# sthagen/kubernetes-kubernetes

Hardware: AMD Instinct MI355X
Metric: pods scheduled/sec + node-evals/sec at 5k/100k nodes, 1/2/4/8 MI355X (higher is better)
Workload: dtype int64; 1 GPU; SchedulingBasic 5000 nodes / 1000 init pods / 491000 measured pods (BASELINE configs[1]); nodes=5000, percentageOfNodesToScore=100, plugins=default, parallelism=single

## Files before the change

### __graft_entry__.py

```python
import os
import subprocess
import sys

ROOT = os.path.dirname(os.path.abspath(__file__))
PKG = os.path.join(ROOT, "kubernetes-kubernetes_amd")
for p in (PKG, os.path.join(ROOT, "tests")):
    if p not in sys.path:
        sys.path.insert(0, p)


def _jobs():
    return str(min(16, os.cpu_count() or 4))


def build() -> None:
    env = dict(os.environ, PYTORCH_ROCM_ARCH="gfx950")
    subprocess.check_call(["make", "-j" + _jobs(), "-C", PKG, "ARCH=gfx950"], env=env)
    subprocess.check_call(["make", "-j" + _jobs(), "-C", os.path.join(ROOT, "oracle")], env=env)
    subprocess.check_call(["make", "-j" + _jobs(), "-C", os.path.join(ROOT, "tests", "asan")], env=env)
    import ksg
    from ksg import native
    native.load()


def smoke() -> None:
    from ksg.native import Scheduler
    from fuzz_gen import rand_cluster, rand_pod
    from oracle_binding import oracle

    rng, cfg, nodes, existing, names = rand_cluster(7, n_nodes=300, n_existing=60, cfg_index=0)
    g = Scheduler(dict(cfg, device=0))
    o = oracle(cfg)
    for b in (g, o):
        for n in nodes:
# ... 20 lines not shown
```

### include/ksg.h

```cpp
#ifndef KSG_H_
#define KSG_H_

#include <stddef.h>
#include <stdint.h>

#ifdef __cplusplus
extern "C" {
#endif

#define KSG_ABI_VERSION 3

#define KSG_OK 0
#define KSG_EINVAL (-1)
#define KSG_ENOTFOUND (-2)
#define KSG_EEXIST (-3)
#define KSG_EDEVICE (-4)
#define KSG_ENOTSUP (-5)
#define KSG_ENOMEM (-6)

#define KSG_CODE_SUCCESS 0
#define KSG_CODE_ERROR 1
#define KSG_CODE_UNSCHEDULABLE 2
#define KSG_CODE_UNSCHEDULABLE_AND_UNRESOLVABLE 3
#define KSG_CODE_WAIT 4
// ... 132 lines not shown

int ksg_debug_relayouts(const ksg_ctx *ctx, uint64_t *full, uint64_t *gather);

int ksg_debug_loop_stats(const ksg_ctx *ctx, uint64_t *give_ups, uint64_t *retries);

int ksg_debug_group_loop_kernel(char *buf, size_t cap);

int ksg_debug_lean_pods(const ksg_ctx *ctx, uint64_t *lean, uint64_t *general);

int ksg_debug_same_pods(const ksg_ctx *ctx, uint64_t *taken, uint64_t *not_taken);

int ksg_debug_compile_memo(const ksg_ctx *ctx, uint64_t *hits, uint64_t *misses);

int ksg_debug_same_carry(const ksg_ctx *ctx, uint64_t *loaded, uint64_t *filled);

int ksg_debug_sched_same(ksg_ctx *ctx, int32_t handle_a, int32_t handle_b);


int ksg_debug_resident_calls(const ksg_ctx *ctx, uint64_t *sched, uint64_t *agg, uint64_t *launch);

int ksg_debug_log_table(double *out, int32_t n);

int ksg_generation(const ksg_ctx *ctx, uint64_t *list_gen, uint64_t *events);

int ksg_debug_schedule_calls(ksg_ctx *ctx, const int32_t *handles, int32_t n, uint32_t flags, ksg_result *results,
                             double *us_per_call);

int ksg_debug_pod_resources(const char *pod_json, size_t len, int64_t *out, int32_t cap);

int ksg_debug_pod_signature(const char *config_json, size_t config_len, const char *pod_json, size_t pod_len, char *out,
// ... 14 lines not shown
```

### kubernetes-kubernetes_amd/csrc/common/desc.h

```cpp
#pragma once
#include <stddef.h>
#include <stdint.h>

#if defined(__HIP__) || defined(__HIPCC__)
#define KSG_HD __host__ __device__
#else
#define KSG_HD
#endif

namespace ksg {

constexpr int kNumPlugins = 10;
constexpr int kBlock = 256;
constexpr int kMaxScalar = 16;
constexpr int kPortSlots = 8;
constexpr int kMaxCons = 32;
constexpr int kMaxPodTerms = 64;
constexpr int kAggMaxCons = 8;
constexpr int kAggMaxTerms = 8;
constexpr int kMaxShards = 8;
constexpr int kBlobLds = 16384;
constexpr int kLoopMaxPods = 1024;
constexpr int kLoopMaxBlk = 2;

// ... 505 lines not shown
  uint32_t* fail;
  unsigned long long* stamps;
  const uint32_t* desc_bytes;
  unsigned long long* wstamps;
  int32_t give_up_at;
  int32_t wave_map;
  PodRing* ring;
  unsigned long long ring_idle;
  int32_t ring_ahead;
  int32_t split_eval;
  int32_t lean_select;
  unsigned long long* relay;
  int32_t* diag;
  unsigned long long* carry;
  uint32_t carry_tag, carry_expect;
};
constexpr int kGran = 16;
constexpr int kFailWords = 16;
constexpr int kFailBytes = kFailWords * 4;

constexpr int kSameScanWaves = 8, kSameCommitWaves = 8;
constexpr int kSameThreads = (kSameScanWaves + kSameCommitWaves) * 64;
constexpr int kSameSlots = 16;
constexpr int kSameMaxNodes = kSameSlots * kSameScanWaves * 64;
constexpr int kSameGroups = kSameMaxNodes / 64;
constexpr int kSameLdsBytes = kBlobLds + kSameMaxNodes * (8 + 1) + kSameGroups * 16 + kLoopMaxPods * (4 + 4 + 16) + 256;
constexpr int kSameSampledLdsBytes = kSameLdsBytes + kLoopMaxPods * (4 + 4) + 64;
static_assert(kSameLdsBytes <= 160 * 1024 && kSameSampledLdsBytes <= 160 * 1024,
              "k_sched_same: one workgroup's LDS (160 KiB per CU on gfx950)");
static_assert(kSameGroups <= 128, "k_sched_same: the group prefix scan holds two groups per lane");
constexpr int kSameCarryTot = 0, kSameCarryFx1 = kSameMaxNodes, kSameCarryBall0 = 2 * kSameMaxNodes,
              kSameCarryBall1 = kSameCarryBall0 + kSameGroups, kSameCarryTagWord = kSameCarryBall1 + kSameGroups;
constexpr int kSameCarryWords = kSameCarryTagWord + 1;
static_assert(kSameMaxNodes >= 5000, "k_sched_same: the flagship workload's nodes fit");

constexpr int kAggThreads = 512;
constexpr int kAggLocal = 4;
constexpr int kAggGWords = 1024;
constexpr int kAggLocalCons = 2;
constexpr int kAggPods = 5120;
constexpr int kAggTerms = 5120;
constexpr int kAggBlobLds = 8192;
// ... 160 lines not shown
```

### kubernetes-kubernetes_amd/csrc/hip/kernels.hip

```cpp
#include <hip/hip_ext.h>
#include <hip/hip_runtime.h>

#include <atomic>
#include <type_traits>

#include "device.hpp"

namespace ksg {

struct NodeCore {
  int64_t acpu, amem, aeph, rcpu, rmem, reph, nzcpu, nzmem;
  int32_t apods, npods;
  uint32_t flags, tlo, thi, ilo, ihi;
};
__device__ __forceinline__ const int32_t* nom_head(const uint8_t* tab) {
  return reinterpret_cast<const int32_t*>(tab + sizeof(NomHdr));
}
template <bool NOM = true>
__device__ __forceinline__ NodeCore load_core(const MirrorView& m, int i) {
  NodeCore c;
  c.acpu = m.alloc_cpu[i];
  c.amem = m.alloc_mem[i];
  c.aeph = m.alloc_eph[i];
  c.rcpu = m.req_cpu[i];
// ... 6525 lines not shown
  int32_t res_node[kLoopMaxPods];
  uint32_t res_F[kLoopMaxPods];
  int32_t slot[kLoopMaxPods], rot[kLoopMaxPods];
  unsigned long long wkey[2][kSameScanWaves];
  uint32_t wnode[2][kSameScanWaves];
  uint32_t arrive, arrive2, done, abort;
  uint8_t pend[kSameMaxNodes];
};
static_assert(sizeof(SameLds) <= (size_t)kSameLdsBytes, "k_sched_same: LDS layout (desc.h kSameLdsBytes)");
struct SameLdsSampled : SameLds {
  uint32_t res_rot[kLoopMaxPods];
  uint32_t res_proc[kLoopMaxPods];
  uint32_t wend[2][kSameScanWaves];
};
static_assert(sizeof(SameLdsSampled) <= (size_t)kSameSampledLdsBytes, "k_sched_same<1>: LDS layout (desc.h kSameSampledLdsBytes)");

__device__ __forceinline__ bool same_wait(SameLds& L, const uint32_t* word, uint32_t want, uint32_t* fail, int q, int what) {
  if ((int32_t)(__hip_atomic_load(word, __ATOMIC_ACQUIRE, __HIP_MEMORY_SCOPE_WORKGROUP) - want) >= 0) return true;
  const unsigned long long t_start = __builtin_amdgcn_s_memrealtime();
  for (uint32_t spins = 1;; ++spins) {
    if ((int32_t)(__hip_atomic_load(word, __ATOMIC_ACQUIRE, __HIP_MEMORY_SCOPE_WORKGROUP) - want) >= 0) return true;
    if ((spins & 63u) == 0u) {
      if (__hip_atomic_load(&L.abort, __ATOMIC_RELAXED, __HIP_MEMORY_SCOPE_WORKGROUP)) return false;
      if (__builtin_amdgcn_s_memrealtime() - t_start > 200000000ull) {
        if ((threadIdx.x & 63) == 0) {
          __hip_atomic_store(&L.abort, 1u, __ATOMIC_RELAXED, __HIP_MEMORY_SCOPE_WORKGROUP);
          __hip_atomic_store(fail + 1, (uint32_t)q, __ATOMIC_RELAXED, __HIP_MEMORY_SCOPE_AGENT);
          __hip_atomic_store(fail + 2, (uint32_t)what, __ATOMIC_RELAXED, __HIP_MEMORY_SCOPE_AGENT);
          __hip_atomic_store(fail + 3, (uint32_t)(threadIdx.x >> 6), __ATOMIC_RELAXED, __HIP_MEMORY_SCOPE_AGENT);
          __hip_atomic_store(fail + 4, 1u, __ATOMIC_RELAXED, __HIP_MEMORY_SCOPE_AGENT);
// ... 49 lines not shown
    for (int g = ct; g < kSameGroups; g += kSameThreads - kScanThreads) {
      cy[kSameCarryBall0 + g] = L.ball0[g];
      cy[kSameCarryBall1 + g] = L.ball1[g];
    }
  }
  __syncthreads();
  if (tid == 0) cy[kSameCarryTagWord] = (unsigned long long)lv.carry_tag;
}

__device__ __forceinline__ NodeEval same_eval(const MirrorView& m, NodeCore c, int k, const PodFast& pf, const uint8_t* base,
                                              const PodDesc& d, int i) {
  for (int a = 0; a < k; ++a) assume_core(c, d);
  return eval_core_fast<false>(m, c, bal2(c.rcpu, c.acpu, c.rmem, c.amem), pf, base, d, i);
}

template <int kSampled>
__global__ __launch_bounds__(kSameThreads) void k_sched_same(MirrorView m_, BatchView b_, LoopView lv_) {
  const LoopGroupArg& ka = *(const LoopGroupArg*)__builtin_amdgcn_kernarg_segment_ptr();
  const MirrorView& m = ka.m;
  const BatchView& b = ka.b;
  const LoopView& lv = ka.lv;
  __shared__ std::conditional_t<kSampled != 0, SameLdsSampled, SameLds> L;
  constexpr int kScanThreads = kSameScanWaves * 64;
  const int tid = (int)threadIdx.x, lane = tid & 63;
  const int wv = __builtin_amdgcn_readfirstlane(tid >> 6);
  const bool scan = wv < kSameScanWaves;
  const int npods = lv.npods;
  loop_entry_record(lv.fail, 0);
  const unsigned long long* cy = lv.carry;
  const bool carried = cy != nullptr && lv.carry_expect != 0u &&
                       (uint32_t)__builtin_amdgcn_readfirstlane((int)(uint32_t)cy[kSameCarryTagWord]) == lv.carry_expect;
  {
    const uint32_t off0 = b.desc_off[lv.first_pod];
    const uint4* src = reinterpret_cast<const uint4*>(b.descs + off0);
    uint4* dst = reinterpret_cast<uint4*>(L.blob);
    const uint32_t n16 = lv.desc_bytes[lv.first_pod] / 16u;
    for (uint32_t o = (uint32_t)tid; o < n16; o += (uint32_t)kSameThreads) dst[o] = src[o];
    for (int k = tid; k < npods; k += kSameThreads) {
      const PodDesc* pd = reinterpret_cast<const PodDesc*>(b.descs + b.desc_off[lv.first_pod + k]);
      L.slot[k] = pd->slot;
      L.rot[k] = pd->rot_start;
    }
    for (int k = tid; k < kSameGroups; k += kSameThreads) {
      L.ball0[k] = carried ? cy[kSameCarryBall0 + k] : 0ull;
      L.ball1[k] = carried ? cy[kSameCarryBall1 + k] : 0ull;
    }
    if (carried)
      for (int k = tid; k < m.n; k += kSameThreads) L.fx1[k] = (int64_t)cy[kSameCarryFx1 + k];
    for (int k = tid; k < kSameMaxNodes; k += kSameThreads) L.pend[k] = 0;
    if (tid == 0) L.arrive = L.arrive2 = L.done = L.abort = 0u;
  }
  __syncthreads();
  if (tid == 0) reinterpret_cast<PodDesc*>(L.blob)->slot = -1;
  __syncthreads();
  const uint8_t* base = L.blob;
  const PodDesc& d = *reinterpret_cast<const PodDesc*>(base);
// ... 25 lines not shown
      if (scan) {
        if constexpr (kSampled) tot[j] = ne.st == 0 ? (uint32_t)(ne.fixed + add) : 0u;
        else key[j] = ne.st == 0 ? pack_best(ne.fixed + add, 0u) : 0ull;
        if (lane == 0) L.ball0[g0 >> 6] = bl;
      } else {
        if (i < n) L.fx1[i] = ne.fixed;
        if (lane == 0) L.ball1[g0 >> 6] = bl;
      }
    }
  }
  __syncthreads();

  if (!scan) {
    const int c = wv - kSameScanWaves;
    for (int q = 0; q < npods; ++q) {
      if (!same_wait(L, &L.done, (uint32_t)(q + 1), lv.fail, q, 2)) return;
      const int node = L.res_node[q];
      if (node >= 0 ? (node % kSameCommitWaves) != c : c != 0) continue;
      if (lane == 0) {
        const int pod = lv.first_pod + q;
        const uint32_t F = L.res_F[q];
        const unsigned long long best = L.res_key[q];
        const int ipa = (int)b.stats[pod].ipa_any;
        if constexpr (kSampled) {
          PodStats* ps = b.stats + pod;
          const uint32_t rot = L.res_rot[q], proc = L.res_proc[q];
          ps->rot = rot;
          ps->processed = proc;
          ps->rot_out = m.n > 0 ? (uint32_t)(((uint64_t)rot + proc) % (uint64_t)m.n) : 0u;
        }
        if (node < 0) {
// ... 178 lines not shown
        dirty = true;
      }
      if (!stays) {
        ++nflip;
        if (lane == 0) __hip_atomic_fetch_add(&L.arrive2, 1u, __ATOMIC_RELEASE, __HIP_MEMORY_SCOPE_WORKGROUP);
        if (!same_wait(L, &L.arrive2, (uint32_t)kSameScanWaves * nflip, lv.fail, q, 1)) return;
        scan_groups();
        reindex();
        dirty = true;
      }
      rot = rot_next;
    }
    same_carry_out<kSampled>(L, lv, n, true, tid, tot);
    return;
  }
  scan_groups();
  rebuild(psb_of(npods > 0 ? L.rot[0] : 0));
  bool dirty = true;
  unsigned long long wk = 0;
  int wn = -1;
  uint32_t wpb = 0;
  uint32_t nflip = 0;
  for (int q = 0; q < npods; ++q) {
    const int par = q & 1;
    const uint32_t psb = psb_of(__builtin_amdgcn_readfirstlane(L.rot[q]));
    if (psb != psb_cur) {
      rebuild(psb);
      dirty = true;
    }
    if (dirty) {
// ... 63 lines not shown
      }
      dirty = true;
    }
    if (!stays) {
      ++nflip;
      if (lane == 0) __hip_atomic_fetch_add(&L.arrive2, 1u, __ATOMIC_RELEASE, __HIP_MEMORY_SCOPE_WORKGROUP);
      if (!same_wait(L, &L.arrive2, (uint32_t)kSameScanWaves * nflip, lv.fail, q, 1)) return;
      scan_groups();
      rebuild(psb_of(__builtin_amdgcn_readfirstlane(L.rot[q + 1 < npods ? q + 1 : q])));
      dirty = true;
    }
  }
  same_carry_out<kSampled>(L, lv, n, true, tid, key);
}
hipError_t launch_sched_same(const MirrorView& m, const BatchView& b, const LoopView& lv, hipStream_t s, hipEvent_t t0,
                             hipEvent_t t1, bool sampled) {
  if (lv.npods < 1 || lv.npods > kLoopMaxPods || m.n > kSameMaxNodes || m.nom != nullptr || lv.ring != nullptr)
    return hipErrorInvalidValue;
  auto* fn = sampled ? k_sched_same<1> : k_sched_same<0>;
  if (t0) hipExtLaunchKernelGGL(fn, dim3(1), dim3(kSameThreads), 0, s, t0, t1, 0, m, b, lv);
  else hipLaunchKernelGGL(fn, dim3(1), dim3(kSameThreads), 0, s, m, b, lv);
  return hipGetLastError();
}

__global__ __launch_bounds__(kBlock) void k_same_diag(MirrorView m, BatchView b, int first_pod, int npods, int32_t* rows) {
  __shared__ __align__(16) uint8_t s_blob[kBlobLds];
  __shared__ DiagLds s_dg;
  __shared__ int s_qf;
  __shared__ uint32_t s_last;
  auto fit_error = [&](int q) {
    const DevResult& r = b.results[first_pod + q];
    return r.feasible == 0 && (r.status == (int32_t)C_UNSCHED || r.status == (int32_t)C_UU);
  };
  if (npods < 1 || !fit_error(npods - 1)) return;
// ... 117 lines not shown
```

### kubernetes-kubernetes_amd/csrc/host/capi.cpp

```cpp
#include <algorithm>
#include <cstring>
#include <memory>
#include <new>
#include <string>

#include "comm.hpp"
#include "host.hpp"

using namespace ksg;

struct ksg_ctx {
  std::unique_ptr<Cluster> cluster;
  std::unique_ptr<Engine> engine;
  std::string err;
};

static thread_local std::string g_create_error;

#define GUARD(body)                                   \
  try {                                               \
    body                                              \
  } catch (const std::bad_alloc&) {                   \
    ctx->err = "out of memory";                       \
    return KSG_ENOMEM;                                \
// ... 552 lines not shown

int ksg_debug_same_pods(const ksg_ctx* ctx, uint64_t* taken, uint64_t* not_taken) {
  if (!ctx || !taken || !not_taken) return KSG_EINVAL;
  *taken = ctx->engine->same_pods_;
  *not_taken = ctx->engine->not_same_pods_;
  return KSG_OK;
}

int ksg_debug_same_carry(const ksg_ctx* ctx, uint64_t* loaded, uint64_t* filled) {
  if (!ctx || !loaded || !filled) return KSG_EINVAL;
  *loaded = ctx->engine->same_carried_;
  *filled = ctx->engine->same_filled_;
  return KSG_OK;
}

int ksg_debug_compile_memo(const ksg_ctx* ctx, uint64_t* hits, uint64_t* misses) {
  if (!ctx || !hits || !misses) return KSG_EINVAL;
  *hits = ctx->engine->memo_hits_;
  *misses = ctx->engine->memo_misses_;
  return KSG_OK;
}

int ksg_debug_sched_same(ksg_ctx* ctx, int32_t handle_a, int32_t handle_b) {
  if (!ctx) return KSG_EINVAL;
  try {
    ksg::Engine* e = ctx->engine.get();
    auto a = e->queue.find(handle_a), b = e->queue.find(handle_b);
    if (a == e->queue.end() || b == e->queue.end()) return KSG_EINVAL;
    ksg::CompiledPod ca, cb;
    int rc = e->compile_full(a->second, ksg::Engine::CYCLE, -1, true, false, &ca, nullptr);
// ... 123 lines not shown
```

### kubernetes-kubernetes_amd/csrc/host/engine.cpp

```cpp
#include <algorithm>
#include <unordered_set>
#include <chrono>
#include <cmath>
#include <cstdlib>
#include <cstdio>
#include <cstring>
#include <cstddef>

#include "comm.hpp"
#include "host.hpp"

namespace ksg {

static bool htrace_on() {
  static const bool on = [] { const char* e = std::getenv("KSG_HOST_TRACE"); return e && *e == '1'; }();
  return on;
}
static thread_local std::string g_htrace;
static void htrace(const char* what, long a = -1) {
  if (!htrace_on()) return;
  static const auto t0 = std::chrono::steady_clock::now();
  char b[96];
  std::snprintf(b, sizeof b, " %.0f:%s%s%ld", std::chrono::duration<double, std::micro>(std::chrono::steady_clock::now() - t0).count(),
                what, a >= 0 ? "=" : "", a >= 0 ? a : 0L);
// ... 17 lines not shown
hipError_t launch_sample_shard_a(const MirrorView& m, const BatchView& b, const ShardView& sv, int pod, hipStream_t s);
hipError_t launch_sample_shard_b(const MirrorView& m, const BatchView& b, const ShardView& sv, int pod, bool cut,
                                 hipStream_t s);
hipError_t launch_unpack_pts(const BatchView& b, const ShardView& sv, int pod, hipStream_t s);
hipError_t launch_xpack_p(const BatchView& b, const ShardView& sv, int pod, hipStream_t s);
hipError_t launch_select_shard(const MirrorView& m, const BatchView& b, const ShardView& sv, int pod, hipStream_t s);
hipError_t launch_commit(const MirrorView& m, const BatchView& b, const ShardView& sv, int pod, hipStream_t s);
#ifdef KSG_DIAG
hipError_t set_diag(unsigned long long* p);
#endif
hipError_t launch_sched_loop(const MirrorView& m, const BatchView& b, const LoopView& lv, hipStream_t s,
                             hipEvent_t t0, hipEvent_t t1, int unit);
hipError_t launch_agg_loop(const MirrorView& m, const BatchView& b, const AggView& av, hipStream_t s, hipEvent_t t0,
                           hipEvent_t t1);
hipError_t launch_sched_same(const MirrorView& m, const BatchView& b, const LoopView& lv, hipStream_t s, hipEvent_t t0,
                             hipEvent_t t1, bool sampled);
hipError_t launch_put_group_arg(const LoopGroupArg& a, LoopGroupArg* dst, hipStream_t s);
hipError_t launch_put_group_arg(const AggGroupArg& a, AggGroupArg* dst, hipStream_t s);
hipError_t launch_sched_loop_group(const LoopGroupArg* ga, int world, int nwg, hipStream_t s, hipEvent_t t0,
                                   hipEvent_t t1, int unit, bool diag, bool nom);
hipError_t launch_agg_loop_group(const AggGroupArg* ga, int world, int nwg, hipStream_t s, hipEvent_t t0, hipEvent_t t1,
                                 bool diag);
hipError_t warm_kernels();
hipError_t warm_aggregate();
hipError_t launch_ob_hint(const MirrorView& m, const BatchView& b, int pod, hipStream_t s);
hipError_t launch_nominated(const MirrorView& m, const BatchView& b, int pod, hipStream_t s);
hipError_t launch_ob_store(const BatchView& b, int pod, hipStream_t s);
hipError_t launch_nom_topo(const MirrorView& m, const BatchView& b, int pod, const PodDesc& d, int nrec, hipStream_t s);
hipError_t launch_filter_score_nt(const MirrorView& m, const BatchView& b, int pod, hipStream_t s, hipEvent_t t0,
                                  hipEvent_t t1, bool lds, int blk0 = 0, int nblk = -1);
hipError_t launch_nominated_shard(const MirrorView& m, const BatchView& b, const ShardView& sv, unsigned long long* xn,
// ... 1190 lines not shown
  if (term_work) b += (double)c->view.n_terms * (double)sizeof(DTerm);
  return b;
}

Engine::~Engine() {
  (void)resident_stop();
  if (ring_) (void)hipHostFree(ring_);
  for (hipEvent_t e : tev) (void)hipEventDestroy(e);
  for (hipEvent_t e : lev) (void)hipEventDestroy(e);
  for (hipEvent_t e : cev) (void)hipEventDestroy(e);
  for (hipEvent_t e : pev) (void)hipEventDestroy(e);
  if (cstream) (void)hipStreamDestroy(cstream);
  for (DevBuf* b : {&d_descs, &d_meta, &d_status, &d_fmask, &d_blk, &d_fixed, &d_raw, &d_out,
                    &d_total, &d_arena, &d_xa, &d_xp, &d_xb, &d_xs, &d_gran, &d_fail, &d_grp, &d_agran, &d_region, &d_astamps, &d_aspill, &d_relay,
                    &d_evg, &d_aggpeers, &d_pre, &d_seg, &d_segcnt, &d_psout, &d_pdb, &d_pick, &d_contrib_buf, &d_wide, &d_vsc,
                    &d_ob, &d_ob_heap, &d_ob_map, &d_tcache, &d_tcw, &d_nom, &d_diag, &d_diag_sum, &d_xn, &d_carry})
    if (b->p) (void)hipFree(b->p);
  if (h_pinned) (void)hipHostFree(h_pinned);
  if (h_tcw) (void)hipHostFree(h_tcw);
  if (h_diag) (void)hipHostFree(h_diag);
  if (ev0) (void)hipEventDestroy(ev0);
  if (ev1) (void)hipEventDestroy(ev1);
}

int Engine::ensure(DevBuf& b, size_t bytes) {
  if (b.bytes >= bytes && b.p) return KSG_OK;
  if (b.p) (void)hipFree(b.p);
  b.p = nullptr;
  b.bytes = 0;
  size_t want = std::max<size_t>(bytes + bytes / 2, 256);
  HIPCHK(hipMalloc(&b.p, want));
// ... 192 lines not shown
  if (!(x.flags & DF_AGGREGATE) || !(y.flags & DF_AGGREGATE) || x.own_terms_off != y.own_terms_off) return false;
  for (PodDesc* z : {&x, &y}) {
    z->slot = 0;
    z->rot_start = 0;
    z->prev_pod = 0;
    z->n_own_terms = 0;
    z->flags &= ~DF_AGG_SAME;
  }
  if (std::memcmp(&x, &y, sizeof(PodDesc)) != 0) return false;
  const size_t end = x.own_terms_off > 0 ? std::min((size_t)x.own_terms_off, a.size()) : a.size();
  return end <= sizeof(PodDesc) ||
         std::memcmp(a.data() + sizeof(PodDesc), b.data() + sizeof(PodDesc), end - sizeof(PodDesc)) == 0;
}

static bool agg_same(const CompiledPod& a, const CompiledPod& b) { return !a.error && !b.error && agg_same(a.blob, b.blob); }

bool Engine::same_eligible(const CompiledPod& p, bool sampled, bool diag) {
  if (p.error || p.blob.size() < sizeof(PodDesc) || p.blob.size() > (size_t)kBlobLds || p.blob.size() % 16 != 0) return false;
  PodDesc d;
  std::memcpy(&d, p.blob.data(), sizeof(PodDesc));
  constexpr uint32_t need = DF_FAST | DF_RAW0 | DF_ASSUME;
  constexpr uint32_t rotating = DF_ROTDEV | DF_SAMPLE;
  constexpr uint32_t never = DF_SUBSET | DF_EARLY | DF_NOM_TOPO | DF_PREFILTER_REJECT |
                             DF_SCORE_ERROR | DF_EVAL_OUT | DF_ALL_FEASIBLE | DF_NODE_LIST | DF_NO_SCORE | DF_AGGREGATE;
  return (d.flags & need) == need && !(d.flags & never) && (sampled || !(d.flags & rotating)) &&
         (diag || !(d.flags & DF_DIAG)) && d.n_pod_ports == 0 && d.n_a_scalar == 0 && d.node_name == -1;
}
static bool same_programs(const CompiledPod& a, const CompiledPod& b) {
  if (a.error || b.error || a.blob.size() != b.blob.size() || a.blob.size() < sizeof(PodDesc)) return false;
  const uint8_t *x = a.blob.data(), *y = b.blob.data();
// ... 942 lines not shown
      bv = bview(n);
    }
    htrace("stage", i);
    r2 = stage(i, b);
    htrace("staged", i);
    return r2;
  };
  const bool same_ok = use_loop && c->cfg.loop_same_template && W == 1 && !comm && m.nom == nullptr &&
                       (!diag || c->cfg.loop_same_diag) && !c->cfg.loop_stamps && c->cfg.debug_give_up_at < 0 &&
                       m.n <= kSameMaxNodes;
  if (same_ok && c->cfg.loop_same_carry) {
    const bool fresh = d_carry.p == nullptr;
    if ((rc = ensure(d_carry, (size_t)kSameCarryWords * 8))) return rc;
    if (fresh) HIPCHK(hipMemsetAsync(d_carry.p, 0, (size_t)kSameCarryWords * 8, s));
  }
  int ss_at = -1, ss_len = 0;
  auto same_stretch = [&](int a, int cut) -> int {
    if (a == ss_at) return ss_len;
    int e = a;
    if (same_eligible(cp[a], c->cfg.loop_same_sampled, c->cfg.loop_same_diag))
      for (e = a + 1; e < n && e < cut && e - a < kLoopMaxPods && same_programs(cp[e - 1], cp[e]);) ++e;
    ss_at = a;
    return ss_len = e - a;
  };
  for (int i = 0; i < n && (!comm || dx);) {
    if (i > 0 && std::binary_search(bnd.begin(), bnd.end(), i) && (chunks.empty() || chunks.back().b < i)) {
      if (i >= compiled && (rc = next_chunk(i))) return rc;
      if ((chunks.empty() || chunks.back().b < i) && (rc = close_chunk(i))) return rc;
    }
    if (cp[i].error) {
// ... 53 lines not shown
        req.la = LoopGroupArg{m, bv, lv};
        req.t0 = t0;
        req.t1 = t1;
        if ((rc = group_launch(&req, false, GS, unit))) return rc;
      } else if (same_run) {
        const bool samp = (reinterpret_cast<const PodDesc*>(cp[i].blob.data())->flags & DF_ROTDEV) != 0;
        if (c->cfg.loop_same_carry) {
          lv.carry = (unsigned long long*)d_carry.p;
          if (++carry_seq_ == 0u) ++carry_seq_;
          lv.carry_tag = carry_seq_;
          const bool load = carry_prev.valid && carry_prev.sampled == samp && same_programs(cp[carry_prev.first], cp[i]);
          lv.carry_expect = load ? carry_prev.tag : 0u;
          ++(load ? same_carried_ : same_filled_);
          carry_prev = CarryPrev{true, i, samp, lv.carry_tag};
        }
        HIPCHK(launch_sched_same(m, bv, lv, s, t0, t1, samp));
        if (diag) HIPCHK(launch_same_diag(m, bv, i, j - i, (int32_t*)d_diag.p, s));
      } else {
        carry_prev.valid = false;
        HIPCHK(launch_sched_loop(m, bv, lv, s, t0, t1, unit));
      }
      runs.push_back({i, j - i, rb, false, tl});
      launches += j - i;
      i = j;
      continue;
    }
    if (use_agg && agg_loop_ok(cp[i])) {
      carry_prev.valid = false;
      int j = i;
      double rb = 0;
      int32_t gw = 1;
// ... 1180 lines not shown
```

### kubernetes-kubernetes_amd/csrc/host/host.hpp

```cpp
#pragma once
#include <hip/hip_runtime.h>

#include <array>
#include <cstdint>
#include <map>
#include <memory>
#include <set>
#include <string>
#include <chrono>
#include <unordered_map>
#include <unordered_set>
#include <vector>

#include "../common/desc.h"
#include "json.hpp"
#include "ksg.h"

namespace ksg {

using StrMap = std::vector<std::pair<std::string, std::string>>;

using Milli = __int128;
constexpr Milli kMilliMax = (Milli)INT64_MAX * 1000;
struct ResAmount {
// ... 157 lines not shown
  bool nominated_evaluate = false;
  bool nominated_all = false;
  bool preempt_nominated_all = false;
  int ring_relay_min = 2;
  int first_chunk = 32;
  int loop_wave_map = 0;
  bool loop_split_eval = true;
  int loop_lean_select = kLeanAll;
  bool loop_same_template = true;
  int loop_same_min_run = 16;
  bool loop_same_sampled = true;
  bool agg_loop_sampled = true;
  bool resident_agg_sampled = true;
  bool loop_same_diag = true;
  bool loop_same_carry = false;
  bool agg_loop_sampled_diag = true;
  int compile_memo = 1;
  bool resident_ahead = true;
  int debug_give_up_at = -1;
  int loop_wg = 0;
  int loop_unit = 128;
  int dev_exchange = -1;
  bool loop_stamps = false;
  int world = 1, rank = 0;
  std::string nccl_id, local_group;
  bool shard_diagnosis = false;
  bool shard_nominations = false;
  bool sharded() const { return world > 1 || !nccl_id.empty() || !local_group.empty(); }
  Config();
};
// ... 281 lines not shown
  int run_batch_api(const std::vector<const PodSpec*>& pods, const std::vector<int32_t>& handles, bool assume,
                    ksg_result* results, ksg_eval_out* eval, ksg_diagnosis* diag = nullptr);
  bool diag_agreed_ = false;
  bool nom_agreed_ = false;
  int fault_first_ = -1;
  bool force_allreduce_ = false;
  uint64_t loop_retries_ = 0;
  uint64_t loop_give_ups_ = 0;
  uint64_t lean_pods_ = 0, general_pods_ = 0;
  void count_lean(const PodDesc& hd) {
    if (!c->cfg.loop_lean_select) return;
    ++((hd.flags & (DF_RAW0 | DF_NO_SCORE)) == DF_RAW0 ? lean_pods_ : general_pods_);
  }
  uint64_t same_pods_ = 0, not_same_pods_ = 0;
  uint64_t same_carried_ = 0, same_filled_ = 0;
  uint32_t carry_seq_ = 0;
  static bool same_eligible(const CompiledPod& p, bool sampled, bool diag = true);
  static bool sched_same(const CompiledPod& a, const CompiledPod& b, bool sampled);
  int run_plugin(const PodSpec& p, Mode mode, int plugin, const uint8_t* nodes, int32_t* code, uint8_t* codes,
                 uint32_t* reasons, int64_t* raw, int64_t* norm);
  int preempt(const PodSpec& p, const char* args_json, size_t args_len, ksg_preempt_result* res, std::string* detail);
  int schedule_resident(const PodSpec& p, int32_t handle, ksg_result* res, bool* handled);
  int resident_stop();

  double algo_bytes(const PodDesc& d) const;
  double agg_bytes(const PodDesc& d) const;
  double last_kernel_ms = 0, last_bytes = 0;
  int32_t last_launches = 0;
  int32_t last_kernel = 0;
  int cu_count = 0;
// ... 31 lines not shown

 private:
  DevBuf d_descs, d_status, d_fmask, d_blk, d_fixed, d_raw, d_out, d_total;
  DevBuf d_ob, d_ob_heap, d_ob_map;
  DevBuf d_meta;
  DevBuf d_off, d_stats, d_results;
  DevBuf d_diag;
  DevBuf d_diag_sum;
  int32_t* h_diag = nullptr;
  size_t h_diag_rows = 0;
  DevBuf d_arena;
  DevBuf d_xa, d_xp, d_xb, d_xs;
  DevBuf d_xn;
  DevBuf d_evg;
  DevBuf d_carry;
  DevBuf d_gran, d_fail, d_stamps;
  uint64_t assume_seq_ = 0;
  DevBuf d_grp;
  struct GroupReq {
    LoopGroupArg la;
    AggGroupArg aa;
    hipEvent_t t0, t1;
  };
  int group_launch(GroupReq* req, bool agg, int nwg, int unit);
  std::vector<unsigned long long*> gran_all;
  uint32_t gran_tag = 0;
  DevBuf d_agran, d_region;
  std::vector<unsigned long long*> agran_all, region_all;
  DevBuf d_aggpeers;
  DevBuf d_astamps;
// ... 52 lines not shown
```

### kubernetes-kubernetes_amd/csrc/host/objects.cpp

```cpp
#include <algorithm>
#include <climits>

#include "host.hpp"

namespace ksg {

bool parse_quantity(const std::string& s, Milli* milli) {
  const char* p = s.c_str();
  const char* e = p + s.size();
  int sign = 1;
  if (p < e && (*p == '+' || *p == '-')) sign = (*p++ == '-') ? -1 : 1;
  unsigned __int128 digits = 0;
  int frac_digits = 0, nd = 0;
  bool seen_dot = false;
  for (; p < e; ++p) {
    if (*p >= '0' && *p <= '9') {
      if (digits > ((unsigned __int128)1 << 96)) return false;
      digits = digits * 10u + (unsigned)(*p - '0');
      nd++;
      if (seen_dot) frac_digits++;
    } else if (*p == '.' && !seen_dot) {
      seen_dot = true;
    } else {
      break;
// ... 917 lines not shown
      return false;
    }
    c->ring_relay_min = (int)d.num(r, "ringRelayMinWorkgroups", 2);
    c->debug_give_up_at = (int)d.num(r, "debugLoopGiveUpAt", -1);
    c->loop_wave_map = (int)d.num(r, "loopWaveMap", 0);
    if (const JVal* se = d.get(r, "loopSplitEval")) c->loop_split_eval = !(se->type == JVal::BOOL && !se->b);
    if (const JVal* ls = d.get(r, "loopLeanSelect"))
      c->loop_lean_select = ls->type == JVal::BOOL ? (ls->b ? kLeanAll : 0) : ((int)d.num(r, "loopLeanSelect", kLeanAll) & kLeanAll);
    if (const JVal* st = d.get(r, "loopSameTemplate")) c->loop_same_template = !(st->type == JVal::BOOL && !st->b);
    c->loop_same_min_run = std::max(1, (int)d.num(r, "loopSameMinRun", c->loop_same_min_run));
    if (const JVal* ss = d.get(r, "loopSameSampled")) c->loop_same_sampled = !(ss->type == JVal::BOOL && !ss->b);
    if (const JVal* as = d.get(r, "aggLoopSampled")) c->agg_loop_sampled = !(as->type == JVal::BOOL && !as->b);
    if (const JVal* rs = d.get(r, "residentAggSampled")) c->resident_agg_sampled = !(rs->type == JVal::BOOL && !rs->b);
    if (const JVal* sd = d.get(r, "loopSameDiag")) c->loop_same_diag = !(sd->type == JVal::BOOL && !sd->b);
    if (const JVal* sc = d.get(r, "loopSameCarry")) c->loop_same_carry = sc->type == JVal::BOOL && sc->b;
    if (const JVal* ad = d.get(r, "aggLoopSampledDiag")) c->agg_loop_sampled_diag = !(ad->type == JVal::BOOL && !ad->b);
    if (const JVal* ra = d.get(r, "residentAhead")) c->resident_ahead = !(ra->type == JVal::BOOL && !ra->b);
    if (d.present(r, "compileMemo")) {
      const std::string cm = d.str(r, "compileMemo");
      if (cm != "on" && cm != "off" && cm != "verify") {
        *err = "compileMemo: Unsupported value \"" + cm + "\" (\"on\", \"off\" or \"verify\")";
        return false;
      }
      c->compile_memo = cm == "off" ? 0 : cm == "on" ? 1 : 2;
    }
    c->first_chunk = std::max(8, std::min(256, (int)d.num(r, "pipelineFirstChunk", 32)));
    if (c->loop_wave_map < 0 || c->loop_wave_map > 2) c->loop_wave_map = 0;
    if (const JVal* dx = d.get(r, "deviceExchange")) c->dev_exchange = dx->type == JVal::BOOL && dx->b ? 1 : 0;
    c->loop_stamps = d.boolean(r, "loopStamps");
    if (const JVal* ds = d.get(r, "distributed")) {
// ... 148 lines not shown
```

### kubernetes-kubernetes_amd/ksg/native.py

```python
import ctypes as C
import os

from .abi import Backend, KsgError

PKG = os.path.dirname(os.path.dirname(os.path.abspath(__file__)))
LIB = os.environ.get("KSG_LIB") or os.path.join(PKG, "lib", "libksg.so")
HEADER = os.path.join(os.path.dirname(PKG), "include", "ksg.h")

_lib = None


def load():
    global _lib
    if _lib is None:
        if not os.path.exists(LIB):
            raise KsgError(f"{LIB} not built: run `make -C {PKG}` or __graft_entry__.build()")
        lib = C.CDLL(LIB)
        lib.ksg_last_batch_kernel_stats.restype = C.c_int
        lib.ksg_last_batch_kernel_stats.argtypes = [C.c_void_p, C.POINTER(C.c_double), C.POINTER(C.c_double),
                                                    C.POINTER(C.c_int32), C.POINTER(C.c_int32)]
        lib.ksg_comm_unique_id.restype = C.c_int
        lib.ksg_comm_unique_id.argtypes = [C.c_char_p, C.c_size_t]
        lib.ksg_create_error.restype = C.c_char_p
        lib.ksg_shard_range.restype = C.c_int
# ... 92 lines not shown
        fn = self.lib.ksg_debug_compile_memo
        fn.restype = C.c_int
        fn.argtypes = [C.c_void_p, C.POINTER(C.c_uint64), C.POINTER(C.c_uint64)]
        a, b = C.c_uint64(), C.c_uint64()
        self._chk(fn(self.ctx, C.byref(a), C.byref(b)), "compile_memo")
        return a.value, b.value

    def same_carry(self):
        fn = self.lib.ksg_debug_same_carry
        fn.restype = C.c_int
        fn.argtypes = [C.c_void_p, C.POINTER(C.c_uint64), C.POINTER(C.c_uint64)]
        a, b = C.c_uint64(), C.c_uint64()
        self._chk(fn(self.ctx, C.byref(a), C.byref(b)), "same_carry")
        return a.value, b.value

    def same_pods(self):
        fn = self.lib.ksg_debug_same_pods
        fn.restype = C.c_int
        fn.argtypes = [C.c_void_p, C.POINTER(C.c_uint64), C.POINTER(C.c_uint64)]
        a, b = C.c_uint64(), C.c_uint64()
        self._chk(fn(self.ctx, C.byref(a), C.byref(b)), "same_pods")
        return a.value, b.value

    def resident_calls(self):
        fn = self.lib.ksg_debug_resident_calls
        fn.restype = C.c_int
        fn.argtypes = [C.c_void_p, C.POINTER(C.c_uint64), C.POINTER(C.c_uint64), C.POINTER(C.c_uint64)]
        a, b, l = C.c_uint64(), C.c_uint64(), C.c_uint64()
        self._chk(fn(self.ctx, C.byref(a), C.byref(b), C.byref(l)), "resident_calls")
        return a.value, b.value, l.value
# ... 53 lines not shown
```

Baseline: 524,300 pods/s.

## Add two-pod lookahead to same-pod scheduling kernel to halve barrier rounds

Adds a k_sched_same<0,1> variant that tracks the top-two keys per scan wave and, when the winning node stays feasible after placement, decides the next pod's placement in the same reduction round. Commit waves now wait per-pod on res_node instead of a shared done counter. The aim is to cut the per-pod cross-wave barrier count in the serial same-pod loop. It costs extra LDS, more register work per round and more complex correctness conditions around rotation and feasibility flips. The build also runs its three make steps in parallel.

```diff
diff --git a/__graft_entry__.py b/__graft_entry__.py
--- a/__graft_entry__.py
+++ b/__graft_entry__.py
@@ -15,9 +15,14 @@
 
 def build() -> None:
     env = dict(os.environ, PYTORCH_ROCM_ARCH="gfx950")
-    subprocess.check_call(["make", "-j" + _jobs(), "-C", PKG, "ARCH=gfx950"], env=env)
-    subprocess.check_call(["make", "-j" + _jobs(), "-C", os.path.join(ROOT, "oracle")], env=env)
-    subprocess.check_call(["make", "-j" + _jobs(), "-C", os.path.join(ROOT, "tests", "asan")], env=env)
+    cmds = [["make", "-j" + _jobs(), "-C", PKG, "ARCH=gfx950"],
+            ["make", "-j" + _jobs(), "-C", os.path.join(ROOT, "oracle")],
+            ["make", "-j" + _jobs(), "-C", os.path.join(ROOT, "tests", "asan")]]
+    procs = [subprocess.Popen(c, env=env) for c in cmds]
+    codes = [p.wait() for p in procs]
+    for c, rc in zip(cmds, codes):
+        if rc:
+            raise subprocess.CalledProcessError(rc, c)
     import ksg
     from ksg import native
     native.load()
diff --git a/include/ksg.h b/include/ksg.h
--- a/include/ksg.h
+++ b/include/ksg.h
@@ -170,6 +170,8 @@
 
 int ksg_debug_same_carry(const ksg_ctx *ctx, uint64_t *loaded, uint64_t *filled);
 
+int ksg_debug_same_lookahead(const ksg_ctx *ctx, uint64_t *own, uint64_t *shared);
+
 int ksg_debug_sched_same(ksg_ctx *ctx, int32_t handle_a, int32_t handle_b);
 
 
diff --git a/kubernetes-kubernetes_amd/csrc/common/desc.h b/kubernetes-kubernetes_amd/csrc/common/desc.h
--- a/kubernetes-kubernetes_amd/csrc/common/desc.h
+++ b/kubernetes-kubernetes_amd/csrc/common/desc.h
@@ -543,6 +543,7 @@
   int32_t* diag;
   unsigned long long* carry;
   uint32_t carry_tag, carry_expect;
+  unsigned long long* look;
 };
 constexpr int kGran = 16;
 constexpr int kFailWords = 16;
@@ -555,6 +556,8 @@
 constexpr int kSameGroups = kSameMaxNodes / 64;
 constexpr int kSameLdsBytes = kBlobLds + kSameMaxNodes * (8 + 1) + kSameGroups * 16 + kLoopMaxPods * (4 + 4 + 16) + 256;
 constexpr int kSameSampledLdsBytes = kSameLdsBytes + kLoopMaxPods * (4 + 4) + 64;
+constexpr int kSameLookLdsBytes = kSameLdsBytes + 2 * kSameScanWaves * 32;
+static_assert(kSameLookLdsBytes <= 160 * 1024, "k_sched_same<0, 1>: one workgroup's LDS");
 static_assert(kSameLdsBytes <= 160 * 1024 && kSameSampledLdsBytes <= 160 * 1024,
               "k_sched_same: one workgroup's LDS (160 KiB per CU on gfx950)");
 static_assert(kSameGroups <= 128, "k_sched_same: the group prefix scan holds two groups per lane");
diff --git a/kubernetes-kubernetes_amd/csrc/hip/kernels.hip b/kubernetes-kubernetes_amd/csrc/hip/kernels.hip
--- a/kubernetes-kubernetes_amd/csrc/hip/kernels.hip
+++ b/kubernetes-kubernetes_amd/csrc/hip/kernels.hip
@@ -6563,6 +6563,11 @@
   uint32_t wend[2][kSameScanWaves];
 };
 static_assert(sizeof(SameLdsSampled) <= (size_t)kSameSampledLdsBytes, "k_sched_same<1>: LDS layout (desc.h kSameSampledLdsBytes)");
+struct SameLdsLook : SameLds {
+  unsigned long long rk1[2][kSameScanWaves], rnk1[2][kSameScanWaves], rk2[2][kSameScanWaves];
+  uint32_t rn1[2][kSameScanWaves], rn2[2][kSameScanWaves];
+};
+static_assert(sizeof(SameLdsLook) <= (size_t)kSameLookLdsBytes, "k_sched_same<0, 1>: LDS layout (desc.h kSameLookLdsBytes)");
 
 __device__ __forceinline__ bool same_wait(SameLds& L, const uint32_t* word, uint32_t want, uint32_t* fail, int q, int what) {
   if ((int32_t)(__hip_atomic_load(word, __ATOMIC_ACQUIRE, __HIP_MEMORY_SCOPE_WORKGROUP) - want) >= 0) return true;
@@ -6642,14 +6647,16 @@
   return eval_core_fast<false>(m, c, bal2(c.rcpu, c.acpu, c.rmem, c.amem), pf, base, d, i);
 }
 
-template <int kSampled>
+template <int kSampled, int kLook = 0>
 __global__ __launch_bounds__(kSameThreads) void k_sched_same(MirrorView m_, BatchView b_, LoopView lv_) {
+  static_assert(!(kSampled && kLook), "k_sched_same: with a cut every pod moves every position, a group is one pod");
   const LoopGroupArg& ka = *(const LoopGroupArg*)__builtin_amdgcn_kernarg_segment_ptr();
   const MirrorView& m = ka.m;
   const BatchView& b = ka.b;
   const LoopView& lv = ka.lv;
-  __shared__ std::conditional_t<kSampled != 0, SameLdsSampled, SameLds> L;
+  __shared__ std::conditional_t<kSampled != 0, SameLdsSampled, std::conditional_t<kLook != 0, SameLdsLook, SameLds>> L;
   constexpr int kScanThreads = kSameScanWaves * 64;
+  constexpr int32_t kNotDecided = -2;
   const int tid = (int)threadIdx.x, lane = tid & 63;
   const int wv = __builtin_amdgcn_readfirstlane(tid >> 6);
   const bool scan = wv < kSameScanWaves;
@@ -6668,6 +6675,7 @@
       const PodDesc* pd = reinterpret_cast<const PodDesc*>(b.descs + b.desc_off[lv.first_pod + k]);
       L.slot[k] = pd->slot;
       L.rot[k] = pd->rot_start;
+      if constexpr (kLook) L.res_node[k] = kNotDecided;
     }
     for (int k = tid; k < kSameGroups; k += kSameThreads) {
       L.ball0[k] = carried ? cy[kSameCarryBall0 + k] : 0ull;
@@ -6723,7 +6731,11 @@
   if (!scan) {
     const int c = wv - kSameScanWaves;
     for (int q = 0; q < npods; ++q) {
-      if (!same_wait(L, &L.done, (uint32_t)(q + 1), lv.fail, q, 2)) return;
+      if constexpr (kLook) {
+        if (!same_wait(L, reinterpret_cast<const uint32_t*>(&L.res_node[q]), 0xffffffffu, lv.fail, q, 4)) return;
+      } else {
+        if (!same_wait(L, &L.done, (uint32_t)(q + 1), lv.fail, q, 2)) return;
+      }
       const int node = L.res_node[q];
       if (node >= 0 ? (node % kSameCommitWaves) != c : c != 0) continue;
       if (lane == 0) {
@@ -6932,6 +6944,174 @@
     same_carry_out<kSampled>(L, lv, n, true, tid, tot);
     return;
   }
+  if constexpr (kLook) {
+    constexpr unsigned long long kPosMask = (1ull << kPreBits) - 1ull;
+    constexpr uint32_t kNoNode = 0x7fffffffu;
+    auto uni64 = [](unsigned long long v) __attribute__((always_inline)) -> unsigned long long {
+      return ((unsigned long long)(uint32_t)__builtin_amdgcn_readfirstlane((int)(uint32_t)(v >> 32)) << 32) |
+             (uint32_t)__builtin_amdgcn_readfirstlane((int)(uint32_t)v);
+    };
+    auto rot_at = [&](int q) __attribute__((always_inline)) -> int { return L.rot[q < npods ? q : npods - 1]; };
+    scan_groups();
+    int rot_cur = npods > 0 ? __builtin_amdgcn_readfirstlane(L.rot[0]) : 0;
+    rebuild(psb_of(rot_cur));
+    bool dirty = true;
+    unsigned long long k1 = 0, nk1 = 0, k2 = 0;
+    uint32_t n1 = kNoNode, n2 = kNoNode;
+    uint32_t nflip = 0, n_own = 0, n_shared = 0;
+    int rot_q = rot_cur, rot_a = npods > 0 ? __builtin_amdgcn_readfirstlane(rot_at(1)) : 0;
+    for (int q = 0, r = 0; q < npods; ++r) {
+      const int par = r & 1;
+      if (rot_q != rot_cur) {
+        const uint32_t psb = psb_of(rot_q);
+        rot_cur = rot_q;
+        if (psb != psb_cur) {
+          rebuild(psb);
+          dirty = true;
+        }
+      }
+      if (dirty) {
+        unsigned long long a = 0, s = 0;
+        int aj = 0, sj = 0;
+#pragma unroll
+        for (int j = 0; j < kSameSlots; ++j) {
+          const unsigned long long kv = key[j];
+          const bool ga = kv > a, gs = kv > s;
+          s = ga ? a : gs ? kv : s;
+          sj = ga ? aj : gs ? j : sj;
+          a = ga ? kv : a;
+          aj = ga ? j : aj;
+        }
+        k1 = wave_max_u64(a);
+        nk1 = k2 = 0ull;
+        n1 = n2 = kNoNode;
+        if (k1 != 0ull) {
+          const int hl = (int)__builtin_ctzll(__ballot(a == k1));
+          const int node1 = __builtin_amdgcn_readlane(aj, hl) * kScanThreads + wv * 64 + hl;
+          const unsigned long long o = lane == hl ? s : a;
+          const int oj = lane == hl ? sj : aj;
+          k2 = wave_max_u64(o);
+          int node2 = -1;
+          if (k2 != 0ull) {
+            const int h2 = (int)__builtin_ctzll(__ballot(o == k2));
+            node2 = __builtin_amdgcn_readlane(oj, h2) * kScanThreads + wv * 64 + h2;
+          }
+          if (!same_wait_pend(L, node1, lv.fail, q)) return;
+          const unsigned long long post1 = ((unsigned long long)(L.fx1[node1] + add) << kPreBits) | (k1 & kPosMask);
+          const uint32_t p1 = (uint32_t)__builtin_amdgcn_readfirstlane((int)((L.ball1[node1 >> 6] >> (node1 & 63)) & 1ull));
+          nk1 = p1 ? uni64(post1) : 0ull;
+          n1 = (uint32_t)node1 | (p1 << 31);
+          if (node2 >= 0) {
+            if (!same_wait_pend(L, node2, lv.fail, q)) return;
+            const uint32_t p2 = (uint32_t)__builtin_amdgcn_readfirstlane((int)((L.ball1[node2 >> 6] >> (node2 & 63)) & 1ull));
+            n2 = (uint32_t)node2 | (p2 << 31);
+          }
+        }
+        dirty = false;
+      }
+      const bool psb_same = rot_a == rot_q || psb_of(rot_a) == psb_cur;
+      if (lane == 0) {
+        L.rk1[par][wv] = k1;
+        L.rnk1[par][wv] = nk1;
+        L.rk2[par][wv] = k2;
+        L.rn1[par][wv] = n1;
+        L.rn2[par][wv] = n2;
+        __hip_atomic_fetch_add(&L.arrive, 1u, __ATOMIC_RELEASE, __HIP_MEMORY_SCOPE_WORKGROUP);
+      }
+      const int rot_b0 = rot_at(q + 2), rot_c0 = rot_at(q + 3);
+      if (!same_wait(L, &L.arrive, (uint32_t)kSameScanWaves * (uint32_t)(r + 1), lv.fail, q, 0)) return;
+      const int rot_b = __builtin_amdgcn_readfirstlane(rot_b0), rot_c = __builtin_amdgcn_readfirstlane(rot_c0);
+      unsigned long long gk = 0, ck = 0;
+      uint32_t gn = kNoNode, cn = kNoNode;
+      int ws = 0;
+#pragma unroll
+      for (int v = 0; v < kSameScanWaves; ++v) {
+        const unsigned long long kv = L.rk1[par][v];
+        const uint32_t nv = L.rn1[par][v];
+        const bool g1 = kv > gk, g2 = kv > ck;
+        ck = g1 ? gk : g2 ? kv : ck;
+        cn = g1 ? gn : g2 ? nv : cn;
+        gk = g1 ? kv : gk;
+        gn = g1 ? nv : gn;
+        ws = g1 ? v : ws;
+      }
+      gk = uni64(gk);
+      gn = (uint32_t)__builtin_amdgcn_readfirstlane((int)gn);
+      if (gk == 0ull) {
+        if (wv == 0 && lane == 0) {
+          L.res_key[q] = 0ull;
+          L.res_F[q] = 0u;
+          __hip_atomic_store(&L.res_node[q], -1, __ATOMIC_RELEASE, __HIP_MEMORY_SCOPE_WORKGROUP);
+        }
+        ++n_own;
+        ++q;
+        rot_q = rot_a;
+        rot_a = rot_b;
+        continue;
+      }
+      auto apply = [&](int qq, unsigned long long wonk, uint32_t nodew, unsigned long long nk) __attribute__((always_inline)) {
+        const int win = (int)(nodew & 0x7fffffffu);
+        const int wslot = win % kScanThreads, wj = win / kScanThreads;
+        const bool me = lane == (wslot & 63);
+#pragma unroll
+        for (int j = 0; j < kSameSlots; ++j) key[j] = me && j == wj ? nk : key[j];
+        if (me) {
+          if (!(nodew >> 31)) L.ball0[win >> 6] &= ~(1ull << (win & 63));
+          L.pend[win] = 1;
+          L.res_key[qq] = wonk;
+          L.res_F[qq] = F;
+          __hip_atomic_store(&L.res_node[qq], win, __ATOMIC_RELEASE, __HIP_MEMORY_SCOPE_WORKGROUP);
+        }
+        dirty = true;
+      };
+      ws = __builtin_amdgcn_readfirstlane(ws);
+      const bool stays = (gn >> 31) != 0u;
+      bool grouped = false, stays2 = true;
+      unsigned long long g2k = 0;
+      uint32_t g2n = kNoNode;
+      bool from_ws = false;
+      if (stays && q + 1 < npods && psb_same) {
+        const unsigned long long nkw = uni64(L.rnk1[par][ws]), k2w = uni64(L.rk2[par][ws]);
+        const uint32_t n2w = (uint32_t)__builtin_amdgcn_readfirstlane((int)L.rn2[par][ws]);
+        ck = uni64(ck);
+        cn = (uint32_t)__builtin_amdgcn_readfirstlane((int)cn);
+        from_ws = k2w > ck;
+        g2k = from_ws ? k2w : ck;
+        g2n = from_ws ? n2w : cn;
+        grouped = g2k > nkw;
+        stays2 = (g2n >> 31) != 0u;
+      }
+      if (ws == wv) apply(q, gk, gn, nk1);
+      if (grouped) {
+        const int win2 = (int)(g2n & 0x7fffffffu);
+        if (((win2 % kScanThreads) >> 6) == wv) {
+          const unsigned long long nk =
+              !from_ws ? nk1 : stays2 ? uni64(((unsigned long long)(L.fx1[win2] + add) << kPreBits) | (g2k & kPosMask)) : 0ull;
+          apply(q + 1, g2k, g2n, nk);
+        }
+        ++n_shared;
+      }
+      ++n_own;
+      q += grouped ? 2 : 1;
+      rot_q = grouped ? rot_b : rot_a;
+      rot_a = grouped ? rot_c : rot_b;
+      if (!stays || !stays2) {
+        ++nflip;
+        if (lane == 0) __hip_atomic_fetch_add(&L.arrive2, 1u, __ATOMIC_RELEASE, __HIP_MEMORY_SCOPE_WORKGROUP);
+        if (!same_wait(L, &L.arrive2, (uint32_t)kSameScanWaves * nflip, lv.fail, q, 1)) return;
+        scan_groups();
+        rot_cur = rot_q;
+        rebuild(psb_of(rot_cur));
+        dirty = true;
+      }
+    }
+    if (lv.look != nullptr && wv == 0 && lane == 0) {
+      __hip_atomic_fetch_add(lv.look + 0, (unsigned long long)n_own, __ATOMIC_RELAXED, __HIP_MEMORY_SCOPE_AGENT);
+      __hip_atomic_fetch_add(lv.look + 1, (unsigned long long)n_shared, __ATOMIC_RELAXED, __HIP_MEMORY_SCOPE_AGENT);
+    }
+    same_carry_out<kSampled>(L, lv, n, true, tid, key);
+    return;
+  }
   scan_groups();
   rebuild(psb_of(npods > 0 ? L.rot[0] : 0));
   bool dirty = true;
@@ -7025,10 +7205,10 @@
   same_carry_out<kSampled>(L, lv, n, true, tid, key);
 }
 hipError_t launch_sched_same(const MirrorView& m, const BatchView& b, const LoopView& lv, hipStream_t s, hipEvent_t t0,
-                             hipEvent_t t1, bool sampled) {
+                             hipEvent_t t1, bool sampled, bool look) {
   if (lv.npods < 1 || lv.npods > kLoopMaxPods || m.n > kSameMaxNodes || m.nom != nullptr || lv.ring != nullptr)
     return hipErrorInvalidValue;
-  auto* fn = sampled ? k_sched_same<1> : k_sched_same<0>;
+  auto* fn = sampled ? k_sched_same<1> : !look ? k_sched_same<0> : k_sched_same<0, 1>;
   if (t0) hipExtLaunchKernelGGL(fn, dim3(1), dim3(kSameThreads), 0, s, t0, t1, 0, m, b, lv);
   else hipLaunchKernelGGL(fn, dim3(1), dim3(kSameThreads), 0, s, m, b, lv);
   return hipGetLastError();
diff --git a/kubernetes-kubernetes_amd/csrc/host/capi.cpp b/kubernetes-kubernetes_amd/csrc/host/capi.cpp
--- a/kubernetes-kubernetes_amd/csrc/host/capi.cpp
+++ b/kubernetes-kubernetes_amd/csrc/host/capi.cpp
@@ -590,6 +590,11 @@
   return KSG_OK;
 }
 
+int ksg_debug_same_lookahead(const ksg_ctx* ctx, uint64_t* own, uint64_t* shared) {
+  if (!ctx || !own || !shared) return KSG_EINVAL;
+  return ctx->engine->same_lookahead(own, shared);
+}
+
 int ksg_debug_compile_memo(const ksg_ctx* ctx, uint64_t* hits, uint64_t* misses) {
   if (!ctx || !hits || !misses) return KSG_EINVAL;
   *hits = ctx->engine->memo_hits_;
diff --git a/kubernetes-kubernetes_amd/csrc/host/engine.cpp b/kubernetes-kubernetes_amd/csrc/host/engine.cpp
--- a/kubernetes-kubernetes_amd/csrc/host/engine.cpp
+++ b/kubernetes-kubernetes_amd/csrc/host/engine.cpp
@@ -55,7 +55,7 @@
 hipError_t launch_agg_loop(const MirrorView& m, const BatchView& b, const AggView& av, hipStream_t s, hipEvent_t t0,
                            hipEvent_t t1);
 hipError_t launch_sched_same(const MirrorView& m, const BatchView& b, const LoopView& lv, hipStream_t s, hipEvent_t t0,
-                             hipEvent_t t1, bool sampled);
+                             hipEvent_t t1, bool sampled, bool look);
 hipError_t launch_put_group_arg(const LoopGroupArg& a, LoopGroupArg* dst, hipStream_t s);
 hipError_t launch_put_group_arg(const AggGroupArg& a, AggGroupArg* dst, hipStream_t s);
 hipError_t launch_sched_loop_group(const LoopGroupArg* ga, int world, int nwg, hipStream_t s, hipEvent_t t0,
@@ -1276,7 +1276,7 @@
   for (DevBuf* b : {&d_descs, &d_meta, &d_status, &d_fmask, &d_blk, &d_fixed, &d_raw, &d_out,
                     &d_total, &d_arena, &d_xa, &d_xp, &d_xb, &d_xs, &d_gran, &d_fail, &d_grp, &d_agran, &d_region, &d_astamps, &d_aspill, &d_relay,
                     &d_evg, &d_aggpeers, &d_pre, &d_seg, &d_segcnt, &d_psout, &d_pdb, &d_pick, &d_contrib_buf, &d_wide, &d_vsc,
-                    &d_ob, &d_ob_heap, &d_ob_map, &d_tcache, &d_tcw, &d_nom, &d_diag, &d_diag_sum, &d_xn, &d_carry})
+                    &d_ob, &d_ob_heap, &d_ob_map, &d_tcache, &d_tcw, &d_nom, &d_diag, &d_diag_sum, &d_xn, &d_carry, &d_look})
     if (b->p) (void)hipFree(b->p);
   if (h_pinned) (void)hipHostFree(h_pinned);
   if (h_tcw) (void)hipHostFree(h_tcw);
@@ -1499,6 +1499,17 @@
 }
 
 static bool agg_same(const CompiledPod& a, const CompiledPod& b) { return !a.error && !b.error && agg_same(a.blob, b.blob); }
+
+int Engine::same_lookahead(uint64_t* own, uint64_t* shared) {
+  *own = *shared = 0;
+  if (d_look.p == nullptr) return KSG_OK;
+  unsigned long long h[2] = {0, 0};
+  HIPCHK(hipMemcpyAsync(h, d_look.p, sizeof h, hipMemcpyDeviceToHost, c->stream));
+  HIPCHK(hipStreamSynchronize(c->stream));
+  *own = h[0];
+  *shared = h[1];
+  return KSG_OK;
+}
 
 bool Engine::same_eligible(const CompiledPod& p, bool sampled, bool diag) {
   if (p.error || p.blob.size() < sizeof(PodDesc) || p.blob.size() > (size_t)kBlobLds || p.blob.size() % 16 != 0) return false;
@@ -2471,6 +2482,10 @@
     if ((rc = ensure(d_carry, (size_t)kSameCarryWords * 8))) return rc;
     if (fresh) HIPCHK(hipMemsetAsync(d_carry.p, 0, (size_t)kSameCarryWords * 8, s));
   }
+  if (same_ok && c->cfg.loop_same_lookahead && d_look.p == nullptr) {
+    if ((rc = ensure(d_look, 2 * 8))) return rc;
+    HIPCHK(hipMemsetAsync(d_look.p, 0, 2 * 8, s));
+  }
   int ss_at = -1, ss_len = 0;
   auto same_stretch = [&](int a, int cut) -> int {
     if (a == ss_at) return ss_len;
@@ -2554,7 +2569,9 @@
           ++(load ? same_carried_ : same_filled_);
           carry_prev = CarryPrev{true, i, samp, lv.carry_tag};
         }
-        HIPCHK(launch_sched_same(m, bv, lv, s, t0, t1, samp));
+        const bool look = c->cfg.loop_same_lookahead && !samp;
+        lv.look = look ? (unsigned long long*)d_look.p : nullptr;
+        HIPCHK(launch_sched_same(m, bv, lv, s, t0, t1, samp, look));
         if (diag) HIPCHK(launch_same_diag(m, bv, i, j - i, (int32_t*)d_diag.p, s));
       } else {
         carry_prev.valid = false;
diff --git a/kubernetes-kubernetes_amd/csrc/host/host.hpp b/kubernetes-kubernetes_amd/csrc/host/host.hpp
--- a/kubernetes-kubernetes_amd/csrc/host/host.hpp
+++ b/kubernetes-kubernetes_amd/csrc/host/host.hpp
@@ -195,6 +195,7 @@
   bool resident_agg_sampled = true;
   bool loop_same_diag = true;
   bool loop_same_carry = false;
+  bool loop_same_lookahead = true;
   bool agg_loop_sampled_diag = true;
   int compile_memo = 1;
   bool resident_ahead = true;
@@ -506,6 +507,7 @@
   }
   uint64_t same_pods_ = 0, not_same_pods_ = 0;
   uint64_t same_carried_ = 0, same_filled_ = 0;
+  int same_lookahead(uint64_t* own, uint64_t* shared);
   uint32_t carry_seq_ = 0;
   static bool same_eligible(const CompiledPod& p, bool sampled, bool diag = true);
   static bool sched_same(const CompiledPod& a, const CompiledPod& b, bool sampled);
@@ -567,6 +569,7 @@
   DevBuf d_xn;
   DevBuf d_evg;
   DevBuf d_carry;
+  DevBuf d_look;
   DevBuf d_gran, d_fail, d_stamps;
   uint64_t assume_seq_ = 0;
   DevBuf d_grp;
diff --git a/kubernetes-kubernetes_amd/csrc/host/objects.cpp b/kubernetes-kubernetes_amd/csrc/host/objects.cpp
--- a/kubernetes-kubernetes_amd/csrc/host/objects.cpp
+++ b/kubernetes-kubernetes_amd/csrc/host/objects.cpp
@@ -955,6 +955,7 @@
     if (const JVal* rs = d.get(r, "residentAggSampled")) c->resident_agg_sampled = !(rs->type == JVal::BOOL && !rs->b);
     if (const JVal* sd = d.get(r, "loopSameDiag")) c->loop_same_diag = !(sd->type == JVal::BOOL && !sd->b);
     if (const JVal* sc = d.get(r, "loopSameCarry")) c->loop_same_carry = sc->type == JVal::BOOL && sc->b;
+    if (const JVal* sl = d.get(r, "loopSameLookahead")) c->loop_same_lookahead = !(sl->type == JVal::BOOL && !sl->b);
     if (const JVal* ad = d.get(r, "aggLoopSampledDiag")) c->agg_loop_sampled_diag = !(ad->type == JVal::BOOL && !ad->b);
     if (const JVal* ra = d.get(r, "residentAhead")) c->resident_ahead = !(ra->type == JVal::BOOL && !ra->b);
     if (d.present(r, "compileMemo")) {
diff --git a/kubernetes-kubernetes_amd/ksg/native.py b/kubernetes-kubernetes_amd/ksg/native.py
--- a/kubernetes-kubernetes_amd/ksg/native.py
+++ b/kubernetes-kubernetes_amd/ksg/native.py
@@ -130,6 +130,14 @@
         self._chk(fn(self.ctx, C.byref(a), C.byref(b)), "same_carry")
         return a.value, b.value
 
+    def same_lookahead(self):
+        fn = self.lib.ksg_debug_same_lookahead
+        fn.restype = C.c_int
+        fn.argtypes = [C.c_void_p, C.POINTER(C.c_uint64), C.POINTER(C.c_uint64)]
+        a, b = C.c_uint64(), C.c_uint64()
+        self._chk(fn(self.ctx, C.byref(a), C.byref(b)), "same_lookahead")
+        return a.value, b.value
+
     def same_pods(self):
         fn = self.lib.ksg_debug_same_pods
         fn.restype = C.c_int
```

New measurement: 573,900 pods/s (median of 4 runs). 1.09x the previous value.
